# tprelle/janusgraph

Hardware: AMD Instinct MI355X
Metric: GTEPS for PageRank iter + BFS, RMAT-24/26, 1/2/4/8 GPUs; % of HBM peak (higher is better)
Workload: dtype f64

## Files before the change

janusgraph_amd/csrc/jg_api.cpp:

```cpp
#include <dlfcn.h>
#include <execinfo.h>

#include <algorithm>
#include <atomic>
#include <cstdlib>
#include <cstring>
#include <limits>
#include <map>
#include <mutex>

#include "jg_cache.h"
#include "jg_internal.h"
#include "jg_labelset.h"

namespace jg {

namespace {
thread_local std::string g_last_error;
}

void rccl_check(ncclResult_t r, const char* what) {
    if (r != ncclSuccess) fail(JG_ERR_RCCL, std::string(what) + ": " + ncclGetErrorString(r));
}

// ... 625 lines not shown
    if (!(cond)) jg::fail(JG_ERR_ARG, msg)

extern "C" {

int jg_abi_version(void) { return JG_ABI_VERSION; }

int jg_tune_set(const char* key, int64_t value) {
    JG_GUARD_BEGIN
    JG_ARG(key, "null key");
    const std::string k(key);
    jg::Tune& t = jg::tune();
    if (k == "dev_poison_probe") {
        jg::dev_poison_probe(value);
        return JG_OK;
    }
    struct Knob {
        const char* name;
        int* field;
        int64_t lo, hi;
    };
    const Knob knobs[] = {
        {"pull_split", &t.pull_split, 0, 1},
        {"halo", &t.halo, 0, 1},
        {"bfs_alpha", &t.bfs_alpha, 1, 1000000},
        {"dobfs_alpha", &t.dobfs_alpha, 1, 1000000},
        {"bfs_beta", &t.bfs_beta, 1, 1000000},
        {"bfs_narrow", &t.bfs_narrow, 0, 1},
        {"nb_alpha", &t.nb_alpha, 1, 1000000},
        {"nb_first", &t.nb_first, 4, 4096},
        {"cc_push", &t.cc_push, 0, 1},
        {"msbfs_sparse", &t.msbfs_sparse, 0, 1},
        {"msbfs_td", &t.msbfs_td, 0, 2},
        {"cc_first", &t.cc_first, 1, 64},
        {"msbfs_skip", &t.msbfs_skip, 0, 1},
        {"msbfs_exit", &t.msbfs_exit, 0, 2},
        {"msbfs_td_rowapply", &t.msbfs_td_rowapply, 0, 1024},
        {"msbfs_td_noprobe", &t.msbfs_td_noprobe, 0, 1000},
        {"msbfs_scan_queue", &t.msbfs_scan_queue, 0, 1001},
        {"msbfs_exit_first", &t.msbfs_exit_first, 1, 256},
        {"msbfs_exit_live", &t.msbfs_exit_live, 0, 1000},
        {"cc_uf", &t.cc_uf, 0, 1},
        {"cc_uf_sharded", &t.cc_uf_sharded, 0, 1},
        {"cc_uf_search", &t.cc_uf_search, 0, 1},
        {"cc_sparse", &t.cc_sparse, 0, 1},
        {"msbfs_split", &t.msbfs_split, 0, 1},
        {"sharded_bfs", &t.sharded_bfs, 0, 1},
        {"bfs_td_split", &t.bfs_td_split, 0, 2},
        {"bfs_td_split_levels", &t.bfs_td_split_levels, 0, 0xffff},
        {"bfs_batch0", &t.bfs_batch0, 1, 64},
        {"bfs_grid_mult", &t.bfs_grid_mult, 1, 64},
        {"bfs_grid", &t.bfs_grid, 64, 65536},
        {"bfs_tail_grid", &t.bfs_tail_grid, 0, 65536},
        {"merge_temporal", &t.merge_temporal, 0, 2},
        {"sd_delta", &t.sd_delta, -1, 1 << 30},
        {"sd_dist32", &t.sd_dist32, 0, 2},
    };
    for (const Knob& kn : knobs) {
        if (k != kn.name) continue;
        if (value < kn.lo || value > kn.hi)
            jg::fail(JG_ERR_ARG, k + " must be in [" + std::to_string(kn.lo) + ", " + std::to_string(kn.hi) + "]");
        *kn.field = (int)value;
        return JG_OK;
    }
    if (k.rfind("band", 0) == 0 && k.size() == 9 && k[4] >= '0' && k[4] <= '3' &&
        (k.substr(5) == "_deg" || k.substr(5) == "_bit" || k.substr(5) == "_sub")) {
        const int i = k[4] - '0';
        if (k.substr(5) == "_deg") {
            JG_ARG(value >= -1, "band degree must be >= 0 (0: unused) or -1 (automatic)");
            t.band_deg[i] = value;
        } else if (k.substr(5) == "_bit") {
            JG_ARG(value == 0 || (value >= 3 && value <= 8), "band bits must be 0 (automatic) or in [3, 8]");
            t.band_bits[i] = value == 0 ? -1 : (int)value;
        } else {
            JG_ARG(value >= 1 && value <= 256 && (value & (value - 1)) == 0, "band sub-slices must be a power of two in [1, 256]");
            int b = 0;
            while ((1 << b) < value) ++b;
            t.band_bits[i] = b;
        }
    } else if (k.size() == 12 && k.compare(0, 11, "merge_stage") == 0 && k[11] >= '0' && k[11] <= '3') {
        JG_ARG(value == -1 || value == 0 || value == 64 || value == 128 || value == 256 || value == 512,
               "merge_stage<i> must be -1 (automatic), 0, 64, 128, 256 or 512");
        t.merge_stage[k[11] - '0'] = (int)value;
    } else if (k == "bfs_td_split_min" || k == "bfs_td_split_max") {
        JG_ARG(value >= 1 && value <= INT32_MAX, "bfs_td_split_min / _max must be in [1, 2^31)");
        (k == "bfs_td_split_min" ? t.bfs_td_split_min : t.bfs_td_split_max) = value;
    } else if (k == "merge_pack") {
        JG_ARG(value == 0 || value == 1 || value == 24, "merge_pack must be 0 (32 bits), 1 (automatic) or 24 (at least 24)");
        t.merge_pack = (int)value;
    } else if (k == "pull_unroll" || k == "pull_nt" || k == "pull_lds" || k == "light_lds" || k == "slice_lds" ||
               k == "pull_short" || k == "pull_overlap" || k == "bfs_persistent") {
    } else {
        jg::fail(JG_ERR_ARG, "unknown tuning key: " + k);
    }
    JG_GUARD_END
}

const char* jg_last_error(void) { return jg::g_last_error.c_str(); }

int jg_comm_unique_id(void* out) {
    JG_GUARD_BEGIN
    JG_ARG(out, "null output");
    ncclUniqueId id;
    jg::rccl_check(ncclGetUniqueId(&id), "ncclGetUniqueId");
    static_assert(sizeof(ncclUniqueId) == JG_UNIQUE_ID_BYTES, "unique id size");
    std::memcpy(out, &id, sizeof id);
    JG_GUARD_END
// ... 834 lines not shown
```

janusgraph_amd/csrc/jg_internal.h:

```cpp
#pragma once

#include <algorithm>
#include <memory>
#include <atomic>
#include <mutex>
#include <functional>
#include <vector>

#include "jg_common.h"
#include "janusgpu.h"

#include <rccl/rccl.h>

namespace jg {

struct Csr {
    int64_t rows = 0;
    int64_t nnz = 0;
    DevBuf<int64_t> row_ptr;
    DevBuf<int32_t> col;
    DevBuf<int32_t> weight;
    mutable int64_t empty_from = -1;
    mutable DevBuf<int32_t> first_col;
    mutable long long wstat[4] = {0, 0, 0, 0};
    mutable bool wstat_ok = false;
    bool present() const { return row_ptr.size() > 0; }
    int64_t bytes() const { return (int64_t)(row_ptr.bytes() + col.bytes() + weight.bytes()); }
};

constexpr int kNumClasses = 9;
constexpr int kZeroClass = kNumClasses - 1;
constexpr int64_t kHubDegree = 8192;
constexpr int kRunMax = 7;
constexpr int64_t kHubChunk = 4096;

struct SliceBand {
    int bits = 3;
    int64_t row_begin = 0, row_end = 0;
    int64_t tasks = 0;
    int64_t subrows = 0;
    int64_t part_off = 0;
    int64_t carry_off = 0;
    DevBuf<int32_t> col;
    int width = 32;
    DevBuf<uint4> pack_a;
    DevBuf<uint32_t> pack_b;
    DevBuf<int64_t> sub_begin;
    DevBuf<int64_t> sub_end;
    DevBuf<int64_t> sub_base;
    DevBuf<uint8_t> heads;
    DevBuf<int32_t> meta;
    DevBuf<uint2> sub_word;
    DevBuf<int32_t> task_rows;
    int64_t rows() const { return row_end - row_begin; }
};

struct PullPlan {
    int64_t class_row_begin[kNumClasses];
    int64_t class_row_end[kNumClasses];
    int64_t class_block_begin[kNumClasses + 1];
    int64_t num_hub_rows = 0;
    int64_t max_hub_row = -1;
    int64_t num_chunks = 0;
    DevBuf<int64_t> chunk_row;
    DevBuf<int64_t> chunk_begin;
    DevBuf<int64_t> chunk_end;
    DevBuf<int64_t> hub_chunk_ptr;
    int64_t total_blocks() const { return class_block_begin[kNumClasses]; }

    int64_t split_rows = 0;
    int64_t col_space = 0;
    int64_t light_row_begin[kNumClasses] = {};
    int64_t light_row_end[kNumClasses] = {};
    int64_t light_block_begin[kNumClasses + 1] = {};
    std::vector<std::unique_ptr<SliceBand>> bands;
    int64_t split_partial_len() const {
        int64_t n = 0;
        for (const auto& b : bands) n += b->subrows + b->tasks;
        return std::max<int64_t>(n, 1);
    }
    bool lds_ok = false;
    bool temporal = false;
    int seg_tbits = 31;
    int nseg = 1;
    bool runs = false;
    int64_t run_begin[kRunMax + 1] = {};
    int64_t run_ptr[kRunMax + 1] = {};
};
constexpr int kXcds = 8;
constexpr int kMergeTask = 512;
__host__ __device__ __forceinline__ uint32_t sub_hash(int64_t c) {
    const uint32_t x = (uint32_t)(c >> 4);
    return (x ^ (x >> 8) ^ (x >> 16) ^ (x >> 24)) & 255u;
}
__host__ __device__ __forceinline__ uint32_t brev_bits(uint32_t v, int bits) {
    uint32_t r = 0;
    for (int i = 0; i < bits; ++i) r |= ((v >> i) & 1u) << (bits - 1 - i);
    return r;
}
__host__ __device__ __forceinline__ uint32_t sub_key(int64_t c) { return brev_bits(sub_hash(c), 8); }
__host__ __device__ __forceinline__ int sub_slice(int64_t c, int bits) { return (int)(sub_hash(c) & ((1u << bits) - 1)); }

struct Ctx;

struct CompactMap {
    const uint32_t* bits = nullptr;
    const int64_t* off = nullptr;
    const int64_t* qbase = nullptr;
    int64_t S = 0;
    int r = 0, tbits = 31;
    __host__ __device__ bool on() const { return bits != nullptr; }
    __device__ __forceinline__ int32_t operator()(int64_t g) const {
        const int64_t q = g / S, l = g - q * S;
        if (q == r) return (int32_t)l;
        const uint32_t w = bits[g >> 5];
        const int64_t rank = off[g >> 5] + __popc(w & ((1u << (g & 31)) - 1u)) - qbase[q];
        return (int32_t)(((q < r ? q + 1 : q) << tbits) + rank);
    }
};

struct Halo {
    bool on = false;
    int tbits = 31;
    int64_t C = 0;
    DevBuf<uint32_t> bits;
    DevBuf<int64_t> off, qbase;
    DevBuf<int32_t> send_src;
    std::vector<int64_t> send_off, recv_off;
    DevBuf<uint64_t> send_buf;
    int seg_of(int q, int r) const { return q < r ? q + 1 : q; }
    CompactMap map(int64_t S, int r) const {
        CompactMap m;
        if (on) { m.bits = bits.get(); m.off = off.get(); m.qbase = qbase.get(); m.S = S; m.r = r; m.tbits = tbits; }
        return m;
    }
};

struct alignas(16) IdSlot {
    unsigned long long key;
    uint32_t val, pad;
};

struct VecPos {
    int64_t base = 0;
    __device__ __forceinline__ int64_t operator()(int64_t row) const { return base + row; }
};

struct Shard {
    int device = 0;
    int index = 0;
    int vtag = -1;
    hipStream_t stream = nullptr;
    ncclComm_t comm = nullptr;
    int64_t rows = 0;
// ... 41 lines not shown
    int sd_hist_n = 0;
    DevBuf<int32_t> kept_depth;
    DevBuf<int32_t> dag_vertex, dag_depth, dag_pred;
    DevBuf<int64_t> dag_off;
    DevBuf<int64_t> census_vid, census_pop;
    std::vector<DevBuf<uint8_t>> nb_level;
    DevBuf<uint8_t> nb_vis;
    DevBuf<unsigned long long> nb_rest;
    DevBuf<int32_t> nb_queue[2];
    DevBuf<int64_t> nb_qoff[2];
    DevBuf<unsigned long long> nb_ctr;
    DevBuf<unsigned char> nb_state;
    DevBuf<const uint8_t*> nb_table;

    std::vector<hipEvent_t> prof_events;
    std::vector<hipEvent_t> exch_events;
    std::vector<int> prof_units;
};

inline bool same_device(const Shard& sh, int dev) { return sh.device == dev && sh.vtag <= 0; }

struct Graph {
    Ctx* ctx = nullptr;
    int64_t n = 0;
    int P = 1;
    int64_t S = 0;
    uint32_t flags = 0;
    std::vector<std::unique_ptr<Shard>> shards;
    DevBuf<IdSlot> id_table;
    int id_dev = 0;
    std::vector<int64_t> vid;
    DevBuf<int32_t> padded_dev;
    mutable std::vector<int32_t> padded_host;
    mutable std::mutex lazy_mu;
    const std::vector<int32_t>& padded_of_dense() const;
    jg_graph_info info{};
    bool has_weights = false;
    int kept_nsrc = 0;
    int kept_dir = 0;
    int64_t dag_nv = -1, dag_ne = 0;
    int64_t census_listed = -1;
    int64_t top_listed = -1;
    std::vector<int64_t> top_index;
    std::vector<double> top_rank, top_edges;
    bool cc_ranks = false;
    DevBuf<int64_t> cc_vor;
    mutable std::vector<int64_t> cc_vor_host;
    const std::vector<int64_t>& vid_of_rank() const;
    int pr_cur = 0;
    bool pr_begun = false;
    double pr_damping = 0.85;
    int64_t pr_vertex_count = 1;
    int pr_steps = 0;

    int64_t vid_of(int64_t dense) const { return vid.empty() ? dense : vid[dense]; }
    int64_t padded_len() const { return (int64_t)P * S; }
    const Halo& halo(const Shard& sh, uint32_t adj) const { return adj == JG_ADJ_BOTH ? sh.halo_both : sh.halo_in; }
    int64_t vec_len(const Shard& sh, uint32_t adj) const {
        const Halo& h = halo(sh, adj);
        return h.on ? std::max<int64_t>(h.C, 1) : padded_len();
    }
    VecPos vec_pos(const Shard& sh, uint32_t adj) const {
        VecPos p;
        p.base = halo(sh, adj).on ? 0 : (int64_t)sh.index * S;
        return p;
    }
};

struct Ctx {
    std::vector<int> devices;
    int nranks = 1;
    int rank = 0;
    bool logical = false;
    bool vdev = false;
    std::vector<ncclComm_t> comms;
    bool host_transport = false;
    jg_transport transport{};
    std::vector<hipStream_t> streams;
    bool profiling = false;
    jg_stats last{};
    std::atomic<int> live{0};
    int total_shards() const { return nranks * (int)devices.size(); }
};

struct DenseEdges {
    std::vector<int32_t*> src, dst;
    std::vector<int32_t*> weight;
    int64_t m = 0;
    bool capped = false, in_from_in = false;
    std::vector<int32_t*> out_src, in_src, in_dst;
    int64_t m_in = 0;
    int64_t truncated_rows = 0;
};
void build_graph_from_dense(Graph& g, DenseEdges& e);
void generate_rmat_device(int scale, uint64_t seed, int64_t m, int32_t* src, int32_t* dst, hipStream_t s);
void remap_ids_device(const int64_t* d_vid, int64_t n, const int64_t* d_src, const int64_t* d_dst, int64_t m,
                      int32_t* dsrc, int32_t* ddst, hipStream_t s, DevBuf<IdSlot>* table = nullptr);
void dense_of_vids(const Graph& g, const int64_t* vids, int64_t k, int64_t* out, int64_t* padded = nullptr);
void mask_ids_device(const int64_t* masked, const int32_t* dense, int64_t m, int32_t* out, hipStream_t s);
void build_pull_plan(Shard& sh, const Csr& csr, PullPlan& plan, int64_t col_space, int64_t vec_entries,
                     int elem_bytes);
int auto_band_bits(int64_t vec_entries, int elem_bytes);

void rccl_check(ncclResult_t r, const char* what);

void exchange_vec(Graph& g, uint32_t adj, std::vector<void*>& bufs, size_t elem_bytes, ncclDataType_t type);
// ... 157 lines not shown
NarrowRun narrow_bfs(Ctx& ctx, Shard& sh, const Csr& push, const Csr& pull, const int64_t* src, int ns, int max_depth,
                     int32_t* planes);
void combine_run(Graph& g, int direction, int combiner, int wrap32, const int64_t* init, int steps, int64_t* out,
                 uint8_t* received_out);

int allreduce_or(Graph& g, int flag);
void allreduce_sum_i64(Graph& g, int64_t* vals, int n);
uint64_t allreduce_or_u64(Graph& g, uint64_t v);

bool pull_split_launches();
bool debug_plan();
bool debug_bfs();

struct Tune {
    int pull_split = 1;
    int64_t band_deg[4] = {96, -1, -1, 0};
    int band_bits[4] = {-1, -1, -1, 3};
    int halo = 1;
    int bfs_alpha = 14;
    int dobfs_alpha = 30;
    int bfs_beta = 24;
    int bfs_narrow = 1;
    int nb_alpha = 30;
    int nb_first = 16;
    int cc_push = 1;
    int msbfs_sparse = 1;
    int msbfs_td = 1;
    int cc_first = 1;
    int msbfs_skip = 1;
    int msbfs_exit = 1;
    int msbfs_td_rowapply = 4;
    int msbfs_td_noprobe = 2;
    int msbfs_scan_queue = 50;
    int msbfs_exit_first = 16;
    int msbfs_exit_live = 950;
    int cc_uf = 1;
    int cc_uf_sharded = 1;
    int cc_uf_search = 1;
    int cc_sparse = 1;
    int msbfs_split = 1;
    int sharded_bfs = 1;
    int bfs_td_split = 2;
    int bfs_td_split_levels = 2;
    int64_t bfs_td_split_min = 65536;
    int64_t bfs_td_split_max = 1 << 20;
    int bfs_batch0 = 10;
    int bfs_grid_mult = 4;
    int bfs_grid = 8192;
    int bfs_tail_grid = 64;
    int sd_dist32 = 1;
    int sd_delta = -1;
    int merge_temporal = 1;
    int merge_stage[4] = {-1, -1, -1, -1};
    int merge_pack = 1;
};
Tune& tune();
void host_allgather(Ctx& c, const void* in, void* out, size_t bytes);
void host_exchange(Ctx& c, const std::vector<int>& speer, const std::vector<const void*>& sbuf,
                   const std::vector<size_t>& sbytes, const std::vector<int>& rpeer, const std::vector<void*>& rbuf,
                   const std::vector<size_t>& rbytes);
int device_cu_count();

bool prof_enabled(const Ctx& c);
void prof_record_start(Ctx& c, Shard& sh);
void prof_record_stop(Ctx& c, Shard& sh, int units = 1);
void prof_collect(Ctx& c, Graph& g);
void exch_record(Ctx& c, Shard& sh);
void prof_discard_exchanges(Graph& g);
struct ExchTimer {
    Graph& g;
    explicit ExchTimer(Graph& gr);
    ~ExchTimer();
};

}

struct jg_ctx {
    jg::Ctx impl;
};
struct jg_graph {
    jg::Graph impl;
    explicit jg_graph(jg::Ctx* c) {
        impl.ctx = c;
        c->live.fetch_add(1);
    }
    ~jg_graph() { impl.ctx->live.fetch_sub(1); }
    jg_graph(const jg_graph&) = delete;
    jg_graph& operator=(const jg_graph&) = delete;
};
```

janusgraph_amd/csrc/jg_pagerank.hip:

```cpp
#include <cstdlib>

#include "jg_pull.h"
#include "jg_scatter.h"

namespace jg {

namespace {

struct PrOp {
    using T = double;
    const double* __restrict__ x;
    double* __restrict__ contrib_out;
    double* __restrict__ rank;
    const int32_t* __restrict__ outdeg;
    VecPos pos;
    double damping, teleport;
    bool write_rank;
    __device__ __forceinline__ double identity() const { return 0.0; }
    __device__ __forceinline__ double combine(double a, double b) const { return __dadd_rn(a, b); }
    __device__ __forceinline__ double gather(int32_t c) const { return x[c]; }
    __device__ __forceinline__ const double* vec() const { return x; }
    __device__ __forceinline__ double shfl_xor(double v, int o) const { return __shfl_xor(v, o, kWave); }
    __device__ __forceinline__ bool active(int64_t) const { return true; }
    __device__ __forceinline__ void finalize(int64_t row, double s) const {
        const double r = __dadd_rn(__dmul_rn(damping, s), teleport);
        if (write_rank) rank[row] = r;
        contrib_out[pos(row)] = r / (double)outdeg[row];
    }
};

__global__ void pr_init_kernel(const int32_t* __restrict__ outdeg, int64_t rows, VecPos pos, double initial,
                               double* __restrict__ contrib, double* __restrict__ rank) {
    for (int64_t l = (int64_t)blockIdx.x * blockDim.x + threadIdx.x; l < rows; l += (int64_t)gridDim.x * blockDim.x) {
        rank[l] = initial;
        contrib[pos(l)] = initial / (double)outdeg[l];
    }
}

void exchange_contrib(Graph& g, int which) {
    std::vector<void*> bufs;
    for (auto& sp : g.shards) bufs.push_back(sp->pr_contrib[which].peer());
    exchange_vec(g, JG_ADJ_IN, bufs, sizeof(double), ncclFloat64);
}

}

void pagerank_begin(Graph& g, double damping, int64_t vertex_count) {
    if (!(g.flags & JG_ADJ_IN)) fail(JG_ERR_UNSUPPORTED, "PageRank needs a graph built with JG_ADJ_IN");
    if (vertex_count == 0) fail(JG_ERR_ARG, "vertexCount must be non-zero");
    for (auto& sp : g.shards) {
        Shard& sh = *sp;
        DeviceGuard dg(sh);
        const int64_t len = g.vec_len(sh, JG_ADJ_IN);
        for (int k = 0; k < 2; ++k) {
            if (sh.pr_contrib[k].size() != (size_t)len) sh.pr_contrib[k].alloc(len);
            JG_HIP(hipMemsetAsync(sh.pr_contrib[k].get(), 0, sh.pr_contrib[k].bytes(), sh.stream));
        }
        if (sh.pr_rank.size() != (size_t)std::max<int64_t>(sh.rows, 1)) {
            const char* f = std::getenv("JG_VDEV_FAULT");
            if (f && *f && *f != '0' && sh.index > 0) {
                DeviceGuard d0(*g.shards[0]);
                sh.pr_rank.alloc(std::max<int64_t>(sh.rows, 1));
            } else {
                sh.pr_rank.alloc(std::max<int64_t>(sh.rows, 1));
            }
        }
        if (sh.pr_hub_partial.size() != (size_t)std::max<int64_t>(sh.plan_in.num_chunks, 1))
            sh.pr_hub_partial.alloc(std::max<int64_t>(sh.plan_in.num_chunks, 1));
        if (sh.pr_split_partial.size() != (size_t)sh.plan_in.split_partial_len()) {
            sh.pr_split_partial.alloc(sh.plan_in.split_partial_len());
        }
        const double initial = 1.0 / (double)vertex_count;
        if (sh.rows > 0) {
            pr_init_kernel<<<grid_for(sh.rows), kBlock, 0, sh.stream>>>(sh.out_degree.get(), sh.rows,
                                                                        g.vec_pos(sh, JG_ADJ_IN), initial,
                                                                        sh.pr_contrib[0].get(), sh.pr_rank.get());
            JG_LAUNCH_CHECK();
        }
    }
    exchange_contrib(g, 0);
    g.pr_cur = 0;
    g.pr_begun = true;
    g.pr_damping = damping;
    g.pr_vertex_count = vertex_count;
    g.pr_steps = 0;
}

void pagerank_steps(Graph& g, int nsteps) {
    if (!g.pr_begun) fail(JG_ERR_STATE, "jg_pagerank_step before jg_pagerank_begin");
    const double teleport = (1.0 - g.pr_damping) / (double)g.pr_vertex_count;
    Ctx* pc = g.ctx->profiling ? g.ctx : nullptr;
    Shard* whole = (pc && g.shards.size() == 1 && g.ctx->total_shards() == 1 && nsteps > 0) ? g.shards[0].get() : nullptr;
    if (whole) {
        DeviceGuard dg(whole->device);
        prof_record_start(*pc, *whole);
        pc = nullptr;
    }
    for (int t = 0; t < nsteps; ++t) {
        const int cur = g.pr_cur, nxt = cur ^ 1;
        for (auto& sp : g.shards) {
            Shard& sh = *sp;
            DeviceGuard dg(sh);
            PrOp op;
            op.x = sh.pr_contrib[cur].get();
            op.contrib_out = sh.pr_contrib[nxt].get();
            op.rank = sh.pr_rank.get();
            op.outdeg = sh.out_degree.get();
            op.pos = g.vec_pos(sh, JG_ADJ_IN);
            op.damping = g.pr_damping;
            op.teleport = teleport;
            op.write_rank = t == nsteps - 1 || g.pr_steps < 2;
            const bool skip_empty = g.pr_steps >= 2;
            launch_pull(sh.in, sh.plan_in, op, sh.pr_hub_partial.get(), sh.stream, pc, &sh, sh.pr_split_partial.get(),
                        skip_empty);
        }
        exchange_contrib(g, nxt);
        g.pr_cur = nxt;
        ++g.pr_steps;
    }
    if (whole) {
        DeviceGuard dg(whole->device);
        prof_record_stop(*g.ctx, *whole, nsteps);
    }
}

void pagerank_end(Graph& g, double* rank_out, double* edge_count_out) {
    if (!g.pr_begun) fail(JG_ERR_STATE, "jg_pagerank_end before jg_pagerank_begin");
    for (auto& sp : g.shards) {
        Shard& sh = *sp;
        DeviceGuard dg(sh);
        JG_HIP(hipStreamSynchronize(sh.stream));
        if (sh.rows == 0) continue;
        if (rank_out) rows_to_dense(g, sh, sh.pr_rank.get(), rank_out);
        if (edge_count_out) rows_to_dense(g, sh, sh.out_degree.get(), edge_count_out);
    }
    prof_collect(*g.ctx, g);
}

}
```

janusgraph_amd/csrc/jg_pull.h:

```cpp
#pragma once

#include <type_traits>

#include "jg_internal.h"
#include "jg_prim.h"

namespace jg {

struct PullArgs {
    const int64_t* __restrict__ row_ptr;
    const int32_t* __restrict__ col;
    const int64_t* __restrict__ chunk_row;
    const int64_t* __restrict__ chunk_begin;
    const int64_t* __restrict__ chunk_end;
    const int64_t* __restrict__ hub_chunk_ptr;
    int64_t num_chunks;
    int64_t num_hub_rows;
    int64_t class_row_begin[kNumClasses];
    int64_t class_row_end[kNumClasses];
    int64_t class_block_begin[kNumClasses + 1];
    int64_t block_offset;
    int64_t skip_rows;
    int runs;
    int64_t run_begin[kRunMax + 1];
// ... 171 lines not shown
                                                         : op.identity();
#pragma unroll
        for (int o = kWave / 2; o > 0; o >>= 1) acc = op.combine(acc, op.shfl_xor(acc, o));
        if (lane_id() == 0) red[wave_id()] = acc;
        __syncthreads();
        if (threadIdx.x == 0) {
            T t = red[0];
#pragma unroll
            for (int w = 1; w < kBlock / kWave; ++w) t = op.combine(t, red[w]);
            hub_partial[b] = t;
        }
        return;
    }
    pull_block_rows<Op, U>(a, op, GlobalGather<Op>{op}, b, (int)threadIdx.x);
}

template <class Op, int U>
__global__ __launch_bounds__(kBlock) void pull_kernel(PullArgs a, Op op, typename Op::T* __restrict__ hub_partial) {
    pull_block<Op, U>(a, op, hub_partial, (int64_t)blockIdx.x + a.block_offset);
}

template <class Op>
__global__ void pull_hub_finalize_kernel(PullArgs a, Op op, const typename Op::T* __restrict__ hub_partial) {
    using T = typename Op::T;
    for (int64_t h = (int64_t)blockIdx.x * blockDim.x + threadIdx.x; h < a.num_hub_rows;
         h += (int64_t)gridDim.x * blockDim.x) {
        const int64_t c0 = a.hub_chunk_ptr[h], c1 = a.hub_chunk_ptr[h + 1];
        if (a.chunk_row[c0] < a.skip_rows) continue;
        T acc = op.identity();
        for (int64_t k = c0; k < c1; ++k) acc = op.combine(acc, hub_partial[k]);
        op.finalize(a.chunk_row[c0], acc);
    }
}

constexpr int kMergeThreads = 1024;
constexpr int kMergeWaves = kMergeThreads / kWave;
constexpr int kMergeEpl = kMergeTask / kWave;
constexpr int kMergeLdsBytes = 160 * 1024;

struct MergeArgs {
    const uint4* __restrict__ pack_a;
    const uint32_t* __restrict__ pack_b;
    const uint8_t* __restrict__ heads;
    const int32_t* __restrict__ meta;
    const int64_t* __restrict__ sub_begin;
    const int64_t* __restrict__ sub_end;
    const int64_t* __restrict__ sub_base;
    int64_t tasks;
    int bits;
    int stage;
    const uint32_t* __restrict__ live;
};

struct HotSegs {
    int32_t hs = 0;
    int tbits = 31;
    int nseg = 1;
};

template <class Op, bool MSEG = true>
struct SliceGather {
    using T = typename Op::T;
    const Op& op;
    lds_ptr<const T> lds;
    uint32_t hg;
    int sb;
    int bits;
    uint32_t hmask, h;
    uint32_t idcell;
    __device__ __forceinline__ bool is_hot(uint32_t loc) const {
        if constexpr (!MSEG) return loc < (hg << 4);
        return ((loc >> 4) & ((1u << sb) - 1u)) < hg;
    }
    __device__ __forceinline__ T hot(uint32_t loc, bool valid) const {
        if constexpr (!MSEG) return lds[valid && loc < (hg << 4) ? loc : idcell];
        const uint32_t g = loc >> 4, j = g & ((1u << sb) - 1u), seg = g >> sb;
        return lds[valid && j < hg ? (((seg * hg + j) << 4) | (loc & 15u)) : idcell];
    }
    __device__ __forceinline__ int32_t col(uint32_t loc) const {
        const uint32_t x = (loc >> 4) << bits;
        const uint32_t hx = (x ^ (x >> 8) ^ (x >> 16) ^ (x >> 24)) & hmask;
        return (int32_t)(((x | (h ^ hx)) << 4) | (loc & 15u));
    }
    __device__ __forceinline__ T cold(uint32_t loc, bool valid, bool lds_on) const {
        T v = op.identity();
        if (valid && !(lds_on && is_hot(loc))) v = op.gather(col(loc));
        return v;
    }
};

template <int W>
__device__ __forceinline__ uint32_t unpack_entry(const uint32_t (&d)[W / 4], int u) {
    const int o = W * u, i = o >> 5, sh = o & 31;
    uint32_t v = d[i] >> sh;
    if (sh + W > 32) v |= d[i + 1] << (32 - sh);
    if constexpr (W < 32) v &= (1u << W) - 1u;
    return v;
}

template <class T>
__device__ __forceinline__ T lane_up(T v, int lane, int d) {
    static_assert(sizeof(T) % 4 == 0, "whole dwords");
    int w[sizeof(T) / 4];
    __builtin_memcpy(w, &v, sizeof(T));
    const int addr = ((lane - d) & (kWave - 1)) << 2;
#pragma unroll
    for (size_t i = 0; i < sizeof(T) / 4; ++i) w[i] = __builtin_amdgcn_ds_bpermute(addr, w[i]);
    __builtin_memcpy(&v, w, sizeof(T));
    return v;
}

template <class Op, class = void>
struct op_task_live : std::false_type {};
template <class Op>
struct op_task_live<Op, std::void_t<decltype(Op::kTaskLive)>> : std::bool_constant<Op::kTaskLive> {};

template <class Op, bool LDS, int PW, bool MSEG = false>
__global__ __launch_bounds__(kMergeThreads) void pull_merge_kernel(MergeArgs a, Op op, typename Op::T* __restrict__ partial,
                                                                   typename Op::T* __restrict__ carry, HotSegs hs,
                                                                   int temporal) {
    using T = typename Op::T;
    extern __shared__ __align__(16) unsigned char merge_lds[];
    const int S = 1 << a.bits;
    const int xs = S < kXcds ? S : kXcds;
    const int rep = kXcds / xs;
    const int per = S / xs;
    const int w = (int)(blockIdx.x >> 3), W = (int)(gridDim.x >> 3);
    const int xcd = (int)(blockIdx.x & (kXcds - 1));
    const int wave = threadIdx.x / kWave, lane = threadIdx.x % kWave;
    lds_ptr<T> hotv = (lds_ptr<T>)merge_lds;
    const int gshift = 4 + a.bits;
    const int hg = hs.hs >> gshift;
    const int nl = hs.nseg * hg;
    lds_ptr<T> stg = hotv + (nl * 16 + 1) + wave * (a.stage + 1);
    lds_ptr<uint32_t> tctr = (lds_ptr<uint32_t>)(hotv + (nl * 16 + 1) + kMergeWaves * (a.stage + 1));
    const int rounds = temporal ? per : 1;
    const uint32_t hmask = (1u << a.bits) - 1u;
    auto image_line = [&](int seg, int j, int hh) {
        const int64_t grp = ((int64_t)seg << (hs.tbits - gshift)) + j;
        return (grp << a.bits) + (int64_t)(hh ^ (sub_hash(grp << gshift) & hmask));
    };
    for (int rd = 0; rd < rounds; ++rd) {
    const int h = (xcd % xs) | ((temporal ? rd : w % per) << 3);
    const int64_t g = (int64_t)(temporal ? w : w / per) * rep + xcd / xs;
    const int64_t G = (int64_t)(temporal ? W : W / per) * rep;
    if constexpr (LDS) {
        if (rd > 0) __syncthreads();
        constexpr int kStage = 8;
        constexpr int kUnit = 16 / (int)sizeof(T);
        static_assert(16 % sizeof(T) == 0 && kUnit <= 16, "16-byte staging units");
        const unsigned char* src = reinterpret_cast<const unsigned char*>(op.vec());
        const int units = nl * 16 / kUnit;
        using u4 = uint32_t __attribute__((ext_vector_type(4)));
        lds_ptr<u4> hv4 = (lds_ptr<u4>)merge_lds;
        for (int q0 = 0; q0 < units; q0 += kStage * kMergeThreads) {
            u4 buf[kStage];
#pragma unroll
            for (int u = 0; u < kStage; ++u) {
                const int q = q0 + u * kMergeThreads + (int)threadIdx.x;
                const int i = q * kUnit, sg = i >> 4;
                int seg = 0, j = sg;
                if (hs.nseg > 1) {
                    seg = sg / hg;
                    j = sg - seg * hg;
                }
                buf[u] = u4{0, 0, 0, 0};
                if (q < units)
                    buf[u] = *reinterpret_cast<const u4*>(src + (image_line(seg, j, h) * 16 + (i & 15)) * (int64_t)sizeof(T));
            }
#pragma unroll
            for (int u = 0; u < kStage; ++u) {
                const int q = q0 + u * kMergeThreads + (int)threadIdx.x;
                if (q < units) hv4[q] = buf[u];
            }
        }
        if (threadIdx.x == 0) {
            hotv[nl * 16] = op.identity();
            *tctr = 0u;
        }
        __syncthreads();
    }
    const SliceGather<Op, MSEG> lg{op,       hotv, (uint32_t)hg, hs.tbits - gshift, a.bits, (1u << a.bits) - 1u, (uint32_t)h,
                             (uint32_t)nl * 16u};
    const int64_t base = a.sub_base[h];
    const int64_t ntask = a.sub_base[h + 1] - base;
    const int64_t hbegin = a.sub_begin[h], hend = a.sub_end[h];
    constexpr bool dyn = LDS;
    const int64_t grot = (g + rd) % G;
    auto task_of = [&](int64_t j) { return j * G + grot; };
    auto grab = [&]() -> int64_t {
        uint32_t j = 0;
        if (lane == 0) j = __hip_atomic_fetch_add(tctr, 1u, __ATOMIC_RELAXED, __HIP_MEMORY_SCOPE_WORKGROUP);
        return task_of((int64_t)__builtin_amdgcn_readfirstlane(j));
    };
    int64_t jstat = wave;
    auto advance = [&]() -> int64_t {
        if (dyn) return grab();
        jstat += kMergeWaves;
        return task_of(jstat);
    };
    auto dead = [&](int64_t kk) -> bool {
        if constexpr (!op_task_live<Op>::value) return false;
        if (a.live == nullptr || kk >= ntask) return false;
        const uint64_t tt = (uint64_t)(base + kk);
        const uint32_t wd = __builtin_amdgcn_readfirstlane(a.live[tt >> 5]);
        return ((wd >> (tt & 31)) & 1u) == 0;
    };
    int64_t k = dyn ? grab() : task_of(jstat);
    while (dead(k)) k = advance();
    if (k >= ntask) continue;
    static_assert(kMergeEpl == 8, "a lane chunk is 8 entries");
    constexpr int DB = PW / 4 - 4;
    auto chunk = [&](int64_t kk) { return (hbegin >> 3) + kk * kWave + lane; };
    auto meta_idx = [&](int64_t kk) { return 2 * (base + kk) + (lane & 1); };
    auto head_idx = [&](int64_t kk) { return (base + kk) * kWave + lane; };
    auto ld = [](const auto* p) { return *p; };
    using v4u = uint32_t __attribute__((ext_vector_type(4)));
    using v2u = uint32_t __attribute__((ext_vector_type(2)));
    auto load_chunk = [&](int64_t kk, uint32_t (&d)[PW / 4]) {
        const int64_t x = chunk(kk);
        const v4u va = ld(reinterpret_cast<const v4u*>(a.pack_a) + x);
        d[0] = va.x, d[1] = va.y, d[2] = va.z, d[3] = va.w;
        if constexpr (DB == 1) {
            d[4] = ld(a.pack_b + x);
        } else if constexpr (DB == 2) {
            const v2u vb = ld(reinterpret_cast<const v2u*>(a.pack_b) + x);
            d[4] = vb.x, d[5] = vb.y;
        } else {
            const v4u vb = ld(reinterpret_cast<const v4u*>(a.pack_b) + x);
            d[4] = vb.x, d[5] = vb.y, d[6] = vb.z, d[7] = vb.w;
        }
    };
    uint32_t cd[PW / 4];
    load_chunk(k, cd);
    uint32_t hb = ld(a.heads + head_idx(k));
    int32_t mw = ld(a.meta + meta_idx(k));
// ... 204 lines not shown
                acc = first ? v[u] : op.combine(acc, v[u]);
                first = false;
            }
#pragma unroll
        for (int u = 0; u < 8; ++u) wc[u] = wn[u];
    }
    op.finalize(r, acc);
}

template <class Op>
__global__ void pull_slice_finalize_kernel(int64_t row0, int64_t rows, Op op, FinalizeBands fb,
                                           const typename Op::T* __restrict__ partial) {
    for (int64_t r = row0 + (int64_t)blockIdx.x * blockDim.x + threadIdx.x; r < rows; r += (int64_t)gridDim.x * blockDim.x)
        slice_finalize_row(r, op, fb, partial);
}

template <class Op, int U>
__global__ __launch_bounds__(kBlock) void pull_light_finalize_kernel(PullArgs a, Op op,
                                                                     typename Op::T* __restrict__ hub_partial,
                                                                     FinalizeBands fb,
                                                                     const typename Op::T* __restrict__ partial,
                                                                     int64_t split_rows, int64_t fin_blocks,
                                                                     int64_t fin_row0) {
    const int64_t b = blockIdx.x;
    if (b < fin_blocks) {
        const int64_t r = fin_row0 + b * kBlock + threadIdx.x;
        if (r < split_rows) slice_finalize_row<Op>(r, op, fb, partial);
        return;
    }
    pull_block<Op, U>(a, op, hub_partial, b - fin_blocks + a.block_offset);
}


template <class Op>
void launch_pull(const Csr& csr, const PullPlan& plan, const Op& op, typename Op::T* hub_partial, hipStream_t s,
                 Ctx* prof_ctx = nullptr, Shard* prof_shard = nullptr, typename Op::T* split_partial = nullptr,
                 bool skip_empty = false, const uint32_t* const* task_live = nullptr, int64_t caller_rows = 0) {
    using T = typename Op::T;
    const bool split = tune().pull_split && plan.split_rows > 0 && split_partial != nullptr;
    if (task_live != nullptr && !op_task_live<Op>::value)
        fail(JG_ERR_UNSUPPORTED, "launch_pull: this Op does not declare kTaskLive");
    size_t band0 = 0;
    if (caller_rows > 0) {
        while (band0 < plan.bands.size() && plan.bands[band0]->row_end <= caller_rows) ++band0;
        if (!split || band0 == 0 || plan.bands[band0 - 1]->row_end != caller_rows)
            fail(JG_ERR_UNSUPPORTED, "launch_pull: caller rows must end a prefix of the split bands");
    }
    PullArgs a = make_pull_args(csr, plan, split);
    if (skip_empty) a.class_block_begin[kNumClasses] = a.class_block_begin[kZeroClass];
    const int64_t blocks = a.class_block_begin[kNumClasses];
    if (prof_ctx) prof_record_start(*prof_ctx, *prof_shard);
    if (split) {
        static bool attr = false;
        if (!attr) {
            JG_HIP(hipFuncSetAttribute((const void*)pull_merge_kernel<Op, true, 20>,
                                       hipFuncAttributeMaxDynamicSharedMemorySize, kMergeLdsBytes));
            JG_HIP(hipFuncSetAttribute((const void*)pull_merge_kernel<Op, true, 24>,
                                       hipFuncAttributeMaxDynamicSharedMemorySize, kMergeLdsBytes));
            JG_HIP(hipFuncSetAttribute((const void*)pull_merge_kernel<Op, true, 32>,
                                       hipFuncAttributeMaxDynamicSharedMemorySize, kMergeLdsBytes));
            JG_HIP(hipFuncSetAttribute((const void*)pull_merge_kernel<Op, true, 20, true>,
                                       hipFuncAttributeMaxDynamicSharedMemorySize, kMergeLdsBytes));
            JG_HIP(hipFuncSetAttribute((const void*)pull_merge_kernel<Op, true, 24, true>,
                                       hipFuncAttributeMaxDynamicSharedMemorySize, kMergeLdsBytes));
            JG_HIP(hipFuncSetAttribute((const void*)pull_merge_kernel<Op, true, 32, true>,
                                       hipFuncAttributeMaxDynamicSharedMemorySize, kMergeLdsBytes));
            attr = true;
        }
        for (size_t bi = band0; bi < plan.bands.size(); ++bi) {
            const SliceBand& bd = *plan.bands[bi];
            if (bd.tasks == 0) continue;
            int stage = tune().merge_stage[std::min<size_t>(bi, 3)];
            if (stage < 0) {
                const double heads = (double)bd.subrows / (double)std::max<int64_t>(bd.tasks, 1);
                stage = 128;
                while (stage < 4.0 * heads && stage < 256) stage *= 2;
            }
            MergeArgs ma{bd.pack_a.get(), bd.pack_b.get(), bd.heads.get(), bd.meta.get(), bd.sub_begin.get(),
                         bd.sub_end.get(), bd.sub_base.get(), bd.tasks, bd.bits, stage,
                         task_live ? task_live[bi] : nullptr};
            T* part = split_partial + bd.part_off;
            T* carry = split_partial + bd.carry_off;
            const int64_t S = 1ll << bd.bits, gsz = 16 * S;
            const unsigned grid = (unsigned)std::max<int64_t>(S, (int64_t)device_cu_count() / S * S);
            const int64_t stage_bytes = (int64_t)kMergeWaves * (stage + 1) * (int64_t)sizeof(T);
            const int64_t hot_max = (int64_t)((kMergeLdsBytes - stage_bytes - 16) / (int64_t)sizeof(T) - 16) * S;
            HotSegs hs;
            hs.tbits = plan.seg_tbits;
            hs.nseg = plan.nseg;
            const int64_t seg_cap = plan.nseg == 1 ? plan.col_space : (1ll << plan.seg_tbits) - gsz;
            hs.hs = plan.lds_ok ? (int32_t)(std::min<int64_t>(hot_max / plan.nseg, seg_cap) / gsz * gsz) : 0;
            const int temporal = tune().merge_temporal == 2 || (tune().merge_temporal == 1 && plan.temporal);
            const size_t lds = hs.hs > 0 ? (size_t)(hs.nseg * (hs.hs / S) + 1) * sizeof(T) + (size_t)stage_bytes + 16 : 0;
            auto go = [&](auto kern) { kern<<<grid, kMergeThreads, lds, s>>>(ma, op, part, carry, hs, temporal); };
            if (hs.hs > 0 && hs.nseg > 1) {
                if (bd.width == 20) go(pull_merge_kernel<Op, true, 20, true>);
                else if (bd.width == 24) go(pull_merge_kernel<Op, true, 24, true>);
                else go(pull_merge_kernel<Op, true, 32, true>);
            } else if (hs.hs > 0) {
                if (bd.width == 20) go(pull_merge_kernel<Op, true, 20>);
                else if (bd.width == 24) go(pull_merge_kernel<Op, true, 24>);
                else go(pull_merge_kernel<Op, true, 32>);
            } else {
                if (bd.width == 20) go(pull_merge_kernel<Op, false, 20>);
                else if (bd.width == 24) go(pull_merge_kernel<Op, false, 24>);
                else go(pull_merge_kernel<Op, false, 32>);
            }
            JG_LAUNCH_CHECK();
        }
        FixupBands fx{};
        for (size_t bi = band0; bi < plan.bands.size(); ++bi) {
            const auto& bp = plan.bands[bi];
            if (fx.n == kMaxBands) fail(JG_ERR_UNSUPPORTED, "too many split bands");
            fx.meta[fx.n] = bp->meta.get();
            fx.part_off[fx.n] = bp->part_off;
            fx.carry_off[fx.n] = bp->carry_off;
            fx.task_begin[fx.n + 1] = fx.task_begin[fx.n] + bp->tasks;
            ++fx.n;
        }
        if (fx.task_begin[fx.n] > 0) {
            pull_merge_fixup_kernel<Op><<<grid_for(fx.task_begin[fx.n], kBlock, 0), kBlock, 0, s>>>(fx, op, split_partial);
            JG_LAUNCH_CHECK();
        }
    }
    auto launch = [&](unsigned grid) {
        pull_kernel<Op, 4><<<grid, kBlock, 0, s>>>(a, op, hub_partial);
        JG_LAUNCH_CHECK();
    };
    FinalizeBands fb{};
    if (split) {
        for (const auto& bp : plan.bands) {
            if (fb.n == kMaxBands) fail(JG_ERR_UNSUPPORTED, "too many split bands");
            fb.sub_word[fb.n] = bp->sub_word.get();
            fb.row_begin[fb.n] = bp->row_begin;
            fb.row_end[fb.n] = bp->row_end;
            fb.part_off[fb.n] = bp->part_off;
            fb.bits[fb.n] = bp->bits;
            ++fb.n;
        }
    }
    const bool fuse = split && !pull_split_launches();
    if (fuse) {
        const int64_t fin_blocks = (plan.split_rows - caller_rows + kBlock - 1) / kBlock;
        const unsigned grid = (unsigned)(fin_blocks + blocks);
        pull_light_finalize_kernel<Op, 4><<<grid, kBlock, 0, s>>>(a, op, hub_partial, fb, split_partial, plan.split_rows,
                                                                  fin_blocks, caller_rows);
        JG_LAUNCH_CHECK();
    } else if (pull_split_launches()) {
// ... 24 lines not shown
```

Before: 386.1.

## Store PageRank contribution vector in slice-major order for split pull merges

Measured after the change: 388.9, median of 6. About the same (+0.7%).

```diff
diff --git a/janusgraph_amd/csrc/jg_api.cpp b/janusgraph_amd/csrc/jg_api.cpp
--- a/janusgraph_amd/csrc/jg_api.cpp
+++ b/janusgraph_amd/csrc/jg_api.cpp
@@ -701,6 +701,7 @@
         {"bfs_grid", &t.bfs_grid, 64, 65536},
         {"bfs_tail_grid", &t.bfs_tail_grid, 0, 65536},
         {"merge_temporal", &t.merge_temporal, 0, 2},
+        {"pr_vec_order", &t.pr_vec_order, 0, 1},
         {"sd_delta", &t.sd_delta, -1, 1 << 30},
         {"sd_dist32", &t.sd_dist32, 0, 2},
     };
diff --git a/janusgraph_amd/csrc/jg_internal.h b/janusgraph_amd/csrc/jg_internal.h
--- a/janusgraph_amd/csrc/jg_internal.h
+++ b/janusgraph_amd/csrc/jg_internal.h
@@ -8,6 +8,7 @@
 #include <vector>
 
 #include "jg_common.h"
+#include "jg_vecorder.h"
 #include "janusgpu.h"
 
 #include <rccl/rccl.h>
@@ -89,17 +90,12 @@
 };
 constexpr int kXcds = 8;
 constexpr int kMergeTask = 512;
-__host__ __device__ __forceinline__ uint32_t sub_hash(int64_t c) {
-    const uint32_t x = (uint32_t)(c >> 4);
-    return (x ^ (x >> 8) ^ (x >> 16) ^ (x >> 24)) & 255u;
-}
 __host__ __device__ __forceinline__ uint32_t brev_bits(uint32_t v, int bits) {
     uint32_t r = 0;
     for (int i = 0; i < bits; ++i) r |= ((v >> i) & 1u) << (bits - 1 - i);
     return r;
 }
 __host__ __device__ __forceinline__ uint32_t sub_key(int64_t c) { return brev_bits(sub_hash(c), 8); }
-__host__ __device__ __forceinline__ int sub_slice(int64_t c, int bits) { return (int)(sub_hash(c) & ((1u << bits) - 1)); }
 
 struct Ctx;
 
@@ -247,6 +243,7 @@
     double pr_damping = 0.85;
     int64_t pr_vertex_count = 1;
     int pr_steps = 0;
+    VecOrder pr_order;
 
     int64_t vid_of(int64_t dense) const { return vid.empty() ? dense : vid[dense]; }
     int64_t padded_len() const { return (int64_t)P * S; }
@@ -510,6 +507,7 @@
     int sd_delta = -1;
     int merge_temporal = 1;
     int merge_stage[4] = {-1, -1, -1, -1};
+    int pr_vec_order = 1;
     int merge_pack = 1;
 };
 Tune& tune();
diff --git a/janusgraph_amd/csrc/jg_pagerank.hip b/janusgraph_amd/csrc/jg_pagerank.hip
--- a/janusgraph_amd/csrc/jg_pagerank.hip
+++ b/janusgraph_amd/csrc/jg_pagerank.hip
@@ -7,8 +7,16 @@
 
 namespace {
 
-struct PrOp {
+template <bool ORD>
+struct PrOrder {
+    VecOrder ord;
+};
+template <>
+struct PrOrder<false> {};
+template <bool ORD>
+struct PrOpT : PrOrder<ORD> {
     using T = double;
+    static constexpr bool kVecOrdered = ORD;
     const double* __restrict__ x;
     double* __restrict__ contrib_out;
     double* __restrict__ rank;
@@ -18,22 +26,30 @@
     bool write_rank;
     __device__ __forceinline__ double identity() const { return 0.0; }
     __device__ __forceinline__ double combine(double a, double b) const { return __dadd_rn(a, b); }
-    __device__ __forceinline__ double gather(int32_t c) const { return x[c]; }
+    __host__ __device__ __forceinline__ VecOrder order() const {
+        if constexpr (ORD) return this->ord;
+        else return VecOrder{};
+    }
+    __device__ __forceinline__ int64_t slot(int64_t c) const {
+        if constexpr (ORD) return this->ord.pos(c);
+        else return c;
+    }
+    __device__ __forceinline__ double gather(int32_t c) const { return x[slot(c)]; }
     __device__ __forceinline__ const double* vec() const { return x; }
     __device__ __forceinline__ double shfl_xor(double v, int o) const { return __shfl_xor(v, o, kWave); }
     __device__ __forceinline__ bool active(int64_t) const { return true; }
     __device__ __forceinline__ void finalize(int64_t row, double s) const {
         const double r = __dadd_rn(__dmul_rn(damping, s), teleport);
         if (write_rank) rank[row] = r;
-        contrib_out[pos(row)] = r / (double)outdeg[row];
+        contrib_out[slot(pos(row))] = r / (double)outdeg[row];
     }
 };
 
-__global__ void pr_init_kernel(const int32_t* __restrict__ outdeg, int64_t rows, VecPos pos, double initial,
+__global__ void pr_init_kernel(const int32_t* __restrict__ outdeg, int64_t rows, VecPos pos, VecOrder ord, double initial,
                                double* __restrict__ contrib, double* __restrict__ rank) {
     for (int64_t l = (int64_t)blockIdx.x * blockDim.x + threadIdx.x; l < rows; l += (int64_t)gridDim.x * blockDim.x) {
         rank[l] = initial;
-        contrib[pos(l)] = initial / (double)outdeg[l];
+        contrib[ord.pos(pos(l))] = initial / (double)outdeg[l];
     }
 }
 
@@ -43,15 +59,45 @@
     exchange_vec(g, JG_ADJ_IN, bufs, sizeof(double), ncclFloat64);
 }
 
+VecOrder choose_order(const Graph& g) {
+    VecOrder row;
+    if (!tune().pr_vec_order || !tune().pull_split) return row;
+    if (g.ctx->total_shards() != 1 || g.shards.size() != 1 || g.P != 1) return row;
+    const Shard& sh = *g.shards[0];
+    const PullPlan& plan = sh.plan_in;
+    if (sh.halo_in.on || plan.nseg != 1 || plan.split_rows <= 0 || plan.bands.empty()) return row;
+    int bits = 0;
+    for (const auto& b : plan.bands) bits = std::max(bits, b->bits);
+    if (bits == 0 || plan.col_space != g.vec_len(sh, JG_ADJ_IN)) return row;
+    const VecOrder vo = make_vec_order(bits, plan.col_space);
+    return vo.fits(sizeof(double)) ? vo : row;
+}
+
+template <bool ORD>
+void pagerank_superstep(Graph& g, Shard& sh, int cur, int nxt, double teleport, bool write_rank, bool skip_empty, Ctx* pc) {
+    PrOpT<ORD> op;
+    op.x = sh.pr_contrib[cur].get();
+    op.contrib_out = sh.pr_contrib[nxt].get();
+    op.rank = sh.pr_rank.get();
+    op.outdeg = sh.out_degree.get();
+    op.pos = g.vec_pos(sh, JG_ADJ_IN);
+    if constexpr (ORD) op.ord = g.pr_order;
+    op.damping = g.pr_damping;
+    op.teleport = teleport;
+    op.write_rank = write_rank;
+    launch_pull(sh.in, sh.plan_in, op, sh.pr_hub_partial.get(), sh.stream, pc, &sh, sh.pr_split_partial.get(), skip_empty);
+}
+
 }
 
 void pagerank_begin(Graph& g, double damping, int64_t vertex_count) {
     if (!(g.flags & JG_ADJ_IN)) fail(JG_ERR_UNSUPPORTED, "PageRank needs a graph built with JG_ADJ_IN");
     if (vertex_count == 0) fail(JG_ERR_ARG, "vertexCount must be non-zero");
+    g.pr_order = choose_order(g);
     for (auto& sp : g.shards) {
         Shard& sh = *sp;
         DeviceGuard dg(sh);
-        const int64_t len = g.vec_len(sh, JG_ADJ_IN);
+        const int64_t len = g.pr_order.padded_len(g.vec_len(sh, JG_ADJ_IN));
         for (int k = 0; k < 2; ++k) {
             if (sh.pr_contrib[k].size() != (size_t)len) sh.pr_contrib[k].alloc(len);
             JG_HIP(hipMemsetAsync(sh.pr_contrib[k].get(), 0, sh.pr_contrib[k].bytes(), sh.stream));
@@ -73,7 +119,7 @@
         const double initial = 1.0 / (double)vertex_count;
         if (sh.rows > 0) {
             pr_init_kernel<<<grid_for(sh.rows), kBlock, 0, sh.stream>>>(sh.out_degree.get(), sh.rows,
-                                                                        g.vec_pos(sh, JG_ADJ_IN), initial,
+                                                                        g.vec_pos(sh, JG_ADJ_IN), g.pr_order, initial,
                                                                         sh.pr_contrib[0].get(), sh.pr_rank.get());
             JG_LAUNCH_CHECK();
         }
@@ -101,18 +147,10 @@
         for (auto& sp : g.shards) {
             Shard& sh = *sp;
             DeviceGuard dg(sh);
-            PrOp op;
-            op.x = sh.pr_contrib[cur].get();
-            op.contrib_out = sh.pr_contrib[nxt].get();
-            op.rank = sh.pr_rank.get();
-            op.outdeg = sh.out_degree.get();
-            op.pos = g.vec_pos(sh, JG_ADJ_IN);
-            op.damping = g.pr_damping;
-            op.teleport = teleport;
-            op.write_rank = t == nsteps - 1 || g.pr_steps < 2;
+            const bool write_rank = t == nsteps - 1 || g.pr_steps < 2;
             const bool skip_empty = g.pr_steps >= 2;
-            launch_pull(sh.in, sh.plan_in, op, sh.pr_hub_partial.get(), sh.stream, pc, &sh, sh.pr_split_partial.get(),
-                        skip_empty);
+            if (g.pr_order.bits) pagerank_superstep<true>(g, sh, cur, nxt, teleport, write_rank, skip_empty, pc);
+            else pagerank_superstep<false>(g, sh, cur, nxt, teleport, write_rank, skip_empty, pc);
         }
         exchange_contrib(g, nxt);
         g.pr_cur = nxt;
diff --git a/janusgraph_amd/csrc/jg_pull.h b/janusgraph_amd/csrc/jg_pull.h
--- a/janusgraph_amd/csrc/jg_pull.h
+++ b/janusgraph_amd/csrc/jg_pull.h
@@ -247,13 +247,18 @@
     const uint32_t* __restrict__ live;
 };
 
+template <class Op, class = void>
+struct op_vec_ordered : std::false_type {};
+template <class Op>
+struct op_vec_ordered<Op, std::void_t<decltype(Op::kVecOrdered)>> : std::bool_constant<Op::kVecOrdered> {};
+
 struct HotSegs {
     int32_t hs = 0;
     int tbits = 31;
     int nseg = 1;
 };
 
-template <class Op, bool MSEG = true>
+template <class Op, bool MSEG = true, int ORD = 0>
 struct SliceGather {
     using T = typename Op::T;
     const Op& op;
@@ -263,6 +268,7 @@
     int bits;
     uint32_t hmask, h;
     uint32_t idcell;
+    const unsigned char* sbase = nullptr;
     __device__ __forceinline__ bool is_hot(uint32_t loc) const {
         if constexpr (!MSEG) return loc < (hg << 4);
         return ((loc >> 4) & ((1u << sb) - 1u)) < hg;
@@ -279,7 +285,11 @@
     }
     __device__ __forceinline__ T cold(uint32_t loc, bool valid, bool lds_on) const {
         T v = op.identity();
-        if (valid && !(lds_on && is_hot(loc))) v = op.gather(col(loc));
+        if (valid && !(lds_on && is_hot(loc))) {
+            if constexpr (ORD == 1) v = *reinterpret_cast<const T*>(sbase + (uint32_t)(loc * (uint32_t)sizeof(T)));
+            else if constexpr (ORD == 2) v = op.vec()[op.order().pos_band(loc, h, bits)];
+            else v = op.gather(col(loc));
+        }
         return v;
     }
 };
@@ -310,11 +320,12 @@
 template <class Op>
 struct op_task_live<Op, std::void_t<decltype(Op::kTaskLive)>> : std::bool_constant<Op::kTaskLive> {};
 
-template <class Op, bool LDS, int PW, bool MSEG = false>
+template <class Op, bool LDS, int PW, bool MSEG = false, int ORD = 0>
 __global__ __launch_bounds__(kMergeThreads) void pull_merge_kernel(MergeArgs a, Op op, typename Op::T* __restrict__ partial,
                                                                    typename Op::T* __restrict__ carry, HotSegs hs,
                                                                    int temporal) {
     using T = typename Op::T;
+    static_assert(ORD == 0 || (op_vec_ordered<Op>::value && !MSEG), "an ordered vector is one segment");
     extern __shared__ __align__(16) unsigned char merge_lds[];
     const int S = 1 << a.bits;
     const int xs = S < kXcds ? S : kXcds;
@@ -339,6 +350,9 @@
     const int h = (xcd % xs) | ((temporal ? rd : w % per) << 3);
     const int64_t g = (int64_t)(temporal ? w : w / per) * rep + xcd / xs;
     const int64_t G = (int64_t)(temporal ? W : W / per) * rep;
+    const unsigned char* sbase = nullptr;
+    if constexpr (ORD == 1)
+        sbase = reinterpret_cast<const unsigned char*>(op.vec()) + op.order().slice_base(h) * (int64_t)sizeof(T);
     if constexpr (LDS) {
         if (rd > 0) __syncthreads();
         constexpr int kStage = 8;
@@ -360,7 +374,13 @@
                     j = sg - seg * hg;
                 }
                 buf[u] = u4{0, 0, 0, 0};
-                if (q < units)
+                if constexpr (ORD == 1) {
+                    if (q < units) buf[u] = *reinterpret_cast<const u4*>(sbase + (uint32_t)q * 16u);
+                } else if constexpr (ORD == 2) {
+                    if (q < units)
+                        buf[u] = *reinterpret_cast<const u4*>(
+                            src + op.order().pos(image_line(seg, j, h) * 16 + (i & 15)) * (int64_t)sizeof(T));
+                } else if (q < units)
                     buf[u] = *reinterpret_cast<const u4*>(src + (image_line(seg, j, h) * 16 + (i & 15)) * (int64_t)sizeof(T));
             }
 #pragma unroll
@@ -375,8 +395,9 @@
         }
         __syncthreads();
     }
-    const SliceGather<Op, MSEG> lg{op,       hotv, (uint32_t)hg, hs.tbits - gshift, a.bits, (1u << a.bits) - 1u, (uint32_t)h,
-                             (uint32_t)nl * 16u};
+    const SliceGather<Op, MSEG, ORD> lg{op,          hotv,           (uint32_t)hg,       hs.tbits - gshift,
+                                        a.bits,      (1u << a.bits) - 1u, (uint32_t)h,   (uint32_t)nl * 16u,
+                                        sbase};
     const int64_t base = a.sub_base[h];
     const int64_t ntask = a.sub_base[h + 1] - base;
     const int64_t hbegin = a.sub_begin[h], hend = a.sub_end[h];
@@ -687,7 +708,22 @@
     if (prof_ctx) prof_record_start(*prof_ctx, *prof_shard);
     if (split) {
         static bool attr = false;
-        if (!attr) {
+        constexpr bool ordered = op_vec_ordered<Op>::value;
+        if constexpr (ordered) {
+            if (plan.nseg != 1) fail(JG_ERR_UNSUPPORTED, "launch_pull: an ordered vector must be one segment");
+            if (!attr) {
+                auto lds_attr = [](auto kern) {
+                    JG_HIP(hipFuncSetAttribute((const void*)kern, hipFuncAttributeMaxDynamicSharedMemorySize, kMergeLdsBytes));
+                };
+                lds_attr(pull_merge_kernel<Op, true, 20, false, 1>);
+                lds_attr(pull_merge_kernel<Op, true, 24, false, 1>);
+                lds_attr(pull_merge_kernel<Op, true, 32, false, 1>);
+                lds_attr(pull_merge_kernel<Op, true, 20, false, 2>);
+                lds_attr(pull_merge_kernel<Op, true, 24, false, 2>);
+                lds_attr(pull_merge_kernel<Op, true, 32, false, 2>);
+                attr = true;
+            }
+        } else if (!attr) {
             JG_HIP(hipFuncSetAttribute((const void*)pull_merge_kernel<Op, true, 20>,
                                        hipFuncAttributeMaxDynamicSharedMemorySize, kMergeLdsBytes));
             JG_HIP(hipFuncSetAttribute((const void*)pull_merge_kernel<Op, true, 24>,
@@ -728,7 +764,29 @@
             const int temporal = tune().merge_temporal == 2 || (tune().merge_temporal == 1 && plan.temporal);
             const size_t lds = hs.hs > 0 ? (size_t)(hs.nseg * (hs.hs / S) + 1) * sizeof(T) + (size_t)stage_bytes + 16 : 0;
             auto go = [&](auto kern) { kern<<<grid, kMergeThreads, lds, s>>>(ma, op, part, carry, hs, temporal); };
-            if (hs.hs > 0 && hs.nseg > 1) {
+            if constexpr (ordered) {
+                const VecOrder vo = op.order();
+                if (bd.bits > vo.bits || !vo.fits(sizeof(T)))
+                    fail(JG_ERR_UNSUPPORTED, "launch_pull: the vector's order does not fit the band");
+                const bool same = bd.bits == vo.bits;
+                auto pick = [&](auto w20, auto w24, auto w32) {
+                    if (bd.width == 20) go(w20);
+                    else if (bd.width == 24) go(w24);
+                    else go(w32);
+                };
+                if (hs.hs > 0 && same)
+                    pick(pull_merge_kernel<Op, true, 20, false, 1>, pull_merge_kernel<Op, true, 24, false, 1>,
+                         pull_merge_kernel<Op, true, 32, false, 1>);
+                else if (hs.hs > 0)
+                    pick(pull_merge_kernel<Op, true, 20, false, 2>, pull_merge_kernel<Op, true, 24, false, 2>,
+                         pull_merge_kernel<Op, true, 32, false, 2>);
+                else if (same)
+                    pick(pull_merge_kernel<Op, false, 20, false, 1>, pull_merge_kernel<Op, false, 24, false, 1>,
+                         pull_merge_kernel<Op, false, 32, false, 1>);
+                else
+                    pick(pull_merge_kernel<Op, false, 20, false, 2>, pull_merge_kernel<Op, false, 24, false, 2>,
+                         pull_merge_kernel<Op, false, 32, false, 2>);
+            } else if (hs.hs > 0 && hs.nseg > 1) {
                 if (bd.width == 20) go(pull_merge_kernel<Op, true, 20, true>);
                 else if (bd.width == 24) go(pull_merge_kernel<Op, true, 24, true>);
                 else go(pull_merge_kernel<Op, true, 32, true>);
diff --git a/janusgraph_amd/csrc/jg_vecorder.h b/janusgraph_amd/csrc/jg_vecorder.h
--- /dev/null
+++ b/janusgraph_amd/csrc/jg_vecorder.h
@@ -0,0 +1,60 @@
+#pragma once
+
+#include <cstdint>
+
+#if defined(__HIPCC__)
+#define JG_VO_FN __host__ __device__ __forceinline__
+#else
+#define JG_VO_FN inline
+#endif
+
+namespace jg {
+
+JG_VO_FN uint32_t sub_hash(int64_t c) {
+    const uint32_t x = (uint32_t)(c >> 4);
+    return (x ^ (x >> 8) ^ (x >> 16) ^ (x >> 24)) & 255u;
+}
+JG_VO_FN int sub_slice(int64_t c, int bits) { return (int)(sub_hash(c) & ((1u << bits) - 1)); }
+
+JG_VO_FN uint32_t band_loc(int64_t c, int bits) { return (uint32_t)(((c >> (4 + bits)) << 4) | (c & 15)); }
+JG_VO_FN int32_t band_col(uint32_t loc, uint32_t h, int bits) {
+    const uint32_t hmask = (1u << bits) - 1u;
+    const uint32_t x = (loc >> 4) << bits;
+    const uint32_t hx = (x ^ (x >> 8) ^ (x >> 16) ^ (x >> 24)) & hmask;
+    return (int32_t)(((x | (h ^ hx)) << 4) | (loc & 15u));
+}
+
+struct VecOrder {
+    int bits = 0;
+    int64_t groups = 0;
+    JG_VO_FN int64_t slice_len() const { return groups << 4; }
+    JG_VO_FN int64_t slice_base(int64_t h) const { return h * (groups << 4); }
+    JG_VO_FN bool fits(int64_t elem_bytes) const {
+        return bits == 0 || (groups < ((int64_t)1 << 24) && slice_len() * elem_bytes < ((int64_t)1 << 32));
+    }
+    JG_VO_FN int64_t pos(int64_t c) const {
+        const uint32_t line = (uint32_t)(c >> 4);
+        const uint32_t slice = sub_hash(c) & ((1u << bits) - 1u) & 255u;
+        const uint32_t g24 = (uint32_t)groups & 0xffffffu;
+        return (int64_t)(((slice * g24 + (line >> bits)) << 4) | ((uint32_t)c & 15u));
+    }
+    JG_VO_FN int64_t pos_band(uint32_t loc, uint32_t h, int b) const {
+        const uint32_t x = (loc >> 4) << b;
+        const uint32_t f = x ^ (x >> 8) ^ (x >> 16) ^ (x >> 24);
+        const uint32_t above = ((1u << bits) - 1u) & ~((1u << b) - 1u);
+        const uint32_t slice = (f & above) | h;
+        const uint32_t group = loc >> (4 + bits - b);
+        return (int64_t)((((slice & 255u) * ((uint32_t)groups & 0xffffffu) + group) << 4) | (loc & 15u));
+    }
+    JG_VO_FN int64_t padded_len(int64_t col_space) const { return bits == 0 ? col_space : (groups << bits) << 4; }
+};
+
+inline VecOrder make_vec_order(int bits, int64_t col_space) {
+    VecOrder o;
+    o.bits = bits;
+    const int64_t lines = (col_space + 15) >> 4;
+    o.groups = (lines + ((int64_t)1 << bits) - 1) >> bits;
+    return o;
+}
+
+}
```
